# knagrecha/saturn

Hardware: NVIDIA H100
Metric: candidate schedules/sec (higher is better)
Workload: dtype f32

## Files before the change

### saturn_b200/csrc/sb_common.cuh

```cuda
#pragma once
#include <cuda_runtime.h>
#include <stdint.h>

#include "../../include/saturn_b200.h"

#if defined(__CUDA_ARCH__) && (__CUDA_ARCH__ != 900)
#error "saturn_b200 kernels target sm_90a (H100) only"
#endif

namespace sb {

constexpr int kSlots = SB_NSLOT;
constexpr int kWarp = 32;
constexpr int kMaxNodes = SB_MAX_NODES;
constexpr float kSentinel = 1.0e6f;

__device__ __forceinline__ float inf_f() { return __int_as_float(0x7f800000); }

__device__ __forceinline__ uint32_t smem_u32(const void* p) {
  return static_cast<uint32_t>(__cvta_generic_to_shared(p));
}
__device__ __forceinline__ uint32_t cluster_ctarank() {
  uint32_t r;
  asm volatile("mov.u32 %0, %%cluster_ctarank;" : "=r"(r));
  return r;
}
__device__ __forceinline__ void cluster_sync_all() {
  asm volatile("barrier.cluster.arrive.release.aligned;" ::: "memory");
  asm volatile("barrier.cluster.wait.acquire.aligned;" ::: "memory");
}
__device__ __forceinline__ uint32_t cluster_map_shared(uint32_t addr, uint32_t rank) {
  uint32_t r;
  asm volatile("mapa.shared::cluster.u32 %0, %1, %2;" : "=r"(r) : "r"(addr), "r"(rank));
  return r;
}

__device__ __forceinline__ void mbar_init(uint64_t* bar, uint32_t count) {
  asm volatile("mbarrier.init.shared::cta.b64 [%0], %1;" ::"r"(smem_u32(bar)), "r"(count) : "memory");
}
__device__ __forceinline__ void mbar_fence_init() {
  asm volatile("fence.mbarrier_init.release.cluster;" ::: "memory");
}
__device__ __forceinline__ void fence_proxy_async() {
  asm volatile("fence.proxy.async.shared::cta;" ::: "memory");
}
__device__ __forceinline__ void mbar_arrive_expect_tx(uint64_t* bar, uint32_t bytes) {
  asm volatile("mbarrier.arrive.expect_tx.shared::cta.b64 _, [%0], %1;" ::"r"(smem_u32(bar)), "r"(bytes)
               : "memory");
}
__device__ __forceinline__ bool mbar_try_wait(uint64_t* bar, uint32_t parity) {
  uint32_t ok;
  asm volatile(
      "{\n\t.reg .pred p;\n\t"
      "mbarrier.try_wait.parity.shared::cta.b64 p, [%1], %2;\n\t"
      "selp.u32 %0, 1, 0, p;\n\t}"
      : "=r"(ok)
      : "r"(smem_u32(bar)), "r"(parity)
      : "memory");
  return ok != 0;
}
__device__ __forceinline__ void mbar_wait(uint64_t* bar, uint32_t parity) {
  uint32_t spins = 0;
  while (!mbar_try_wait(bar, parity)) {
    if (++spins > (1u << 26)) __trap();
  }
}
__device__ __forceinline__ void tma_bulk_g2s(void* dst_smem, const void* src_gmem, uint32_t bytes,
                                             uint64_t* bar) {
  asm volatile(
      "cp.async.bulk.shared::cluster.global.mbarrier::complete_tx::bytes [%0], [%1], %2, [%3];" ::"r"(
          smem_u32(dst_smem)),
      "l"(src_gmem), "r"(bytes), "r"(smem_u32(bar))
      : "memory");
}

__device__ __forceinline__ void pmov_fma(float& dst, float src, int bit, int one) {
  int d = __float_as_int(dst);
  asm("{\n\t.reg .pred p;\n\tsetp.ne.s32 p, %2, 0;\n\t@p mad.lo.s32 %0, %1, %3, 0;\n\t}"
      : "+r"(d)
      : "r"(__float_as_int(src)), "r"(bit), "r"(one));
  dst = __int_as_float(d);
}
__device__ __forceinline__ void pinf_fma(float& dst, int bit) {
  asm("{\n\t.reg .pred p;\n\tsetp.ne.s32 p, %1, 0;\n\t@p add.f32 %0, %0, 0f7F800000;\n\t}" : "+f"(dst) : "r"(bit));
}
__device__ __forceinline__ float psel(float a, float b, int bit) {
  float r;
  asm("{\n\t.reg .pred p;\n\tsetp.ne.s32 p, %3, 0;\n\tselp.f32 %0, %1, %2, p;\n\t}" : "=f"(r) : "f"(a), "f"(b), "r"(bit));
  return r;
}

__device__ __forceinline__ float fmax3(float a, float b, float c) { return fmaxf(fmaxf(a, b), c); }

template <bool kIntegerStarts, bool kTrackMk = kIntegerStarts>
__device__ __forceinline__ void ls_step(float (&f)[8], float& mk, float& pend, float rt, int km1, int one, int ph) {
  const float INF = inf_f();
  const int b2 = km1 & 4, b1 = km1 & 2, b0 = km1 & 1;
  float x0 = psel(f[4], f[0], b2), x1 = psel(f[5], f[1], b2), x2 = psel(f[6], f[2], b2), x3 = psel(f[7], f[3], b2);
  const float m2 = psel(INF, -0.0f, b2);
  float x4 = f[4] + m2, x5 = f[5] + m2, x6 = f[6] + m2, x7 = f[7] + m2;
  pmov_fma(x0, x2, b1, one); pmov_fma(x1, x3, b1, one); pmov_fma(x2, x4, b1, one); pmov_fma(x3, x5, b1, one);
  pmov_fma(x4, x6, b1, one); pmov_fma(x5, x7, b1, one); pinf_fma(x6, b1); pinf_fma(x7, b1);
  pmov_fma(x0, x1, b0, one); pmov_fma(x1, x2, b0, one); pmov_fma(x2, x3, b0, one); pmov_fma(x3, x4, b0, one);
  pmov_fma(x4, x5, b0, one); pmov_fma(x5, x6, b0, one); pmov_fma(x6, x7, b0, one); pinf_fma(x7, b0);
  const float s = x0;
  float v;
  if (kIntegerStarts) {
    v = s + ceilf(rt);
  } else {
    v = s + rt;
  }
  if (kTrackMk) {
    const float e = kIntegerStarts ? s + rt : v;
    if (ph < 0) mk = fmaxf(mk, e);
    else if (ph == 0) pend = e;
    else mk = fmax3(mk, pend, e);
  }
  f[0] = fmaxf(f[0], fminf(v, x1));
  f[1] = fmaxf(f[1], fminf(v, x2));
  f[2] = fmaxf(f[2], fminf(v, x3));
  f[3] = fmaxf(f[3], fminf(v, x4));
  f[4] = fmaxf(f[4], fminf(v, x5));
  f[5] = fmaxf(f[5], fminf(v, x6));
  f[6] = fmaxf(f[6], fminf(v, x7));
  f[7] = fmaxf(f[7], v);
}

__device__ __forceinline__ unsigned long long pack_key(float mk, uint32_t id) {
  return (static_cast<unsigned long long>(__float_as_uint(mk)) << 32) | id;
}

__device__ __host__ __forceinline__ uint64_t mix64(uint64_t z) {
  z += 0x9e3779b97f4a7c15ull;
  z = (z ^ (z >> 30)) * 0xbf58476d1ce4e5b9ull;
  z = (z ^ (z >> 27)) * 0x94d049bb133111ebull;
  return z ^ (z >> 31);
}
__device__ __host__ __forceinline__ uint64_t rng_u64(uint64_t seed, uint64_t stream, uint64_t ctr) {
  return mix64(mix64(seed ^ (stream * 0xd1342543de82ef95ull)) + ctr * 0x2545f4914f6cdd1dull);
}

}
```

### saturn_b200/csrc/sb_eval.cu

```cuda
#include "sb_lane.cuh"

namespace sb {

struct TileArgs {
  const float* tab;
  int J, SG;
  const uint8_t* opt;
  const uint8_t* prio;
  long long B;
  long long stride_o, stride_p;
  int row_o, row_p;
  int copy_o, copy_p;
  int use_bulk;
  int nodes;
  float* out;
  unsigned long long* best_key;
  uint32_t id_base;
  long long ntiles;
  int one;
  SearchFuse sf;
  XchgPost xp;
};

template <int PB, bool INT, bool STREAM, bool MULTI, bool SEARCH = false, bool TABG = false, int ADDR = 0>
__global__ void __launch_bounds__(STREAM ? 512 : 384, 1) k_eval_tiles(const TileArgs a) {
  static_assert(!(SEARCH && (STREAM || TABG)), "the fused search round runs on shared-memory tiles only");
  static_assert(ADDR == 0 || (!TABG && !MULTI && !SEARCH), "ADDR = 1 needs the table and the opt rows in shared memory");
  extern __shared__ __align__(128) uint8_t smem[];
  const int nw = blockDim.x >> 5;
  const int warp = threadIdx.x >> 5, lane = threadIdx.x & 31;
  const uint32_t tab_bytes = TABG ? 0u : static_cast<uint32_t>(a.J) * a.SG * 4u;
  float* tab_s = reinterpret_cast<float*>(smem);
  uint64_t* bars = reinterpret_cast<uint64_t*>(smem + ((tab_bytes + 15u) & ~15u));
  uint8_t* tiles = reinterpret_cast<uint8_t*>(bars) + (((1 + nw) * 8 + 15) & ~15);
  const uint32_t node_bytes = MULTI ? static_cast<uint32_t>(a.nodes) * 1024u : 0u;
  const uint32_t tile_bytes = 32u * (a.row_o + (STREAM ? 0 : a.row_p)) + node_bytes;
  uint8_t* wbase = tiles + static_cast<size_t>(warp) * tile_bytes;
  float4* node_s = reinterpret_cast<float4*>(wbase);
  uint8_t* tile_o = wbase + node_bytes;
  uint8_t* tile_p = tile_o + 32u * a.row_o;
  uint64_t* bar_tab = bars;
  uint64_t* bar_w = bars + 1 + warp;

  if (threadIdx.x == 0) {
    mbar_init(bar_tab, 1);
    for (int w = 0; w < nw; ++w) mbar_init(bars + 1 + w, 1);
    mbar_fence_init();
  }
  __syncthreads();
  if constexpr (!TABG) {
    if (threadIdx.x == 0) {
      mbar_arrive_expect_tx(bar_tab, tab_bytes);
      const uint8_t* src = reinterpret_cast<const uint8_t*>(a.tab);
      for (uint32_t off = 0; off < tab_bytes; off += 32768u) {
        uint32_t n = min(32768u, tab_bytes - off);
        tma_bulk_g2s(smem + off, src + off, n, bar_tab);
      }
    }
  }

  LaneState<INT, MULTI, ADDR> st;
  if (TABG) st.tab = a.tab;
  else st.tab = tab_s;
  st.SG = a.SG;
  st.one = a.one;
  st.orow = tile_o + lane * a.row_o;
  st.ns = node_s + lane;
  st.orow_s = smem_u32(tile_o + lane * a.row_o);
  st.tab_s = smem_u32(tab_s);
  st.four = static_cast<uint32_t>(a.one) * 4u;

  bool fold_pending = a.xp.counter != nullptr && a.xp.fold_prev && a.xp.seq > 1 && blockIdx.x == 0 && warp == 0;
  unsigned long long pf_seen = 0ull, pf_key = ~0ull;
  auto look_issue = [&]() {
    if (lane < a.xp.x.world) {
      const unsigned long long* slot = a.xp.x.peer[lane] + ((a.xp.seq - 1) & 1ull) * 2;
      asm volatile("ld.acquire.sys.global.u64 %0, [%1];" : "=l"(pf_seen) : "l"(slot + 1) : "memory");
      asm volatile("ld.relaxed.sys.global.u64 %0, [%1];" : "=l"(pf_key) : "l"(slot) : "memory");
    }
  };
  auto fold_keys = [&](unsigned long long k) {
#pragma unroll
    for (int d = 16; d > 0; d >>= 1) {
      const unsigned long long o = __shfl_xor_sync(0xffffffffu, k, d);
      k = o < k ? o : k;
    }
    if (lane == 0) atomicMin(a.best_key, k);
    fold_pending = false;
  };
  auto look_consume = [&]() {
    const unsigned long long want = a.xp.seq - 1;
    const bool ok = lane >= a.xp.x.world || pf_seen >= want;
    if (__all_sync(0xffffffffu, ok)) fold_keys(lane < a.xp.x.world ? pf_key : ~0ull);
  };
  auto try_fold = [&](bool block) {
    const unsigned long long want = a.xp.seq - 1;
    unsigned long long k = ~0ull;
    bool ok = true;
    if (lane < a.xp.x.world) {
      const unsigned long long* slot = a.xp.x.peer[lane] + (want & 1ull) * 2;
      unsigned long long seen;
      unsigned spins = 0;
      for (;;) {
        asm volatile("ld.acquire.sys.global.u64 %0, [%1];" : "=l"(seen) : "l"(slot + 1) : "memory");
        if (seen >= want || !block || ++spins >= (1u << 22)) break;
        __nanosleep(64);
      }
      ok = seen >= want;
      if (ok) asm volatile("ld.relaxed.sys.global.u64 %0, [%1];" : "=l"(k) : "l"(slot) : "memory");
    }
    ok = __all_sync(0xffffffffu, ok);
    if (!ok) {
      if (block && lane == 0) *a.xp.error = 1;
      return;
    }
    fold_keys(k);
  };
  if (fold_pending) look_issue();

  uint32_t phase = 0;
  bool tab_ready = TABG;
  for (long long tile = static_cast<long long>(blockIdx.x) * nw + warp; tile < a.ntiles;
       tile += static_cast<long long>(gridDim.x) * nw) {
    const long long b0 = tile * 32;
    if (!SEARCH && fold_pending) {
      look_consume();
      if (fold_pending) look_issue();
    }
    const long long cand = (SEARCH && a.sf.deal) ? lane * a.ntiles + tile : b0 + lane;
    const bool active = cand < a.B;
    const int nb = SEARCH ? __popc(__ballot_sync(0xffffffffu, active)) : static_cast<int>(min(32ll, a.B - b0));
    const uint8_t* pg = a.prio + cand * a.stride_p;
    __syncwarp();
    PrioChunk q;
    if (a.use_bulk) {
      fence_proxy_async();
      if (lane == 0)
        mbar_arrive_expect_tx(bar_w, static_cast<uint32_t>(nb) * (a.copy_o + (STREAM ? 0 : a.copy_p)));
      __syncwarp();
      if (active) {
        tma_bulk_g2s(tile_o + lane * a.row_o, a.opt + cand * a.stride_o, a.copy_o, bar_w);
        if (!STREAM) tma_bulk_g2s(tile_p + lane * a.row_p, pg, a.copy_p, bar_w);
      }
      if (STREAM && active) q = ld_prio32<true>(pg);
      mbar_wait(bar_w, phase);
      phase ^= 1;
    } else {
      for (int r = 0; r < nb; ++r) {
        const uint8_t* so = a.opt + (b0 + r) * a.stride_o;
        const uint8_t* sp = a.prio + (b0 + r) * a.stride_p;
        for (int x = lane; x < a.J; x += 32) tile_o[r * a.row_o + x] = so[x];
        for (int x = lane; x < a.J * PB; x += 32) tile_p[r * a.row_p + x] = sp[x];
      }
      __syncwarp();
    }
    if (!tab_ready) {
      mbar_wait(bar_tab, 0);
      tab_ready = true;
    }
    auto evaluate = [&](const uint8_t* prio_row_s) -> float {
      st.reset(a.nodes);
      const int J = a.J;
      if (STREAM) {
        constexpr int STEPS = 32 / PB;
        const int nch = (J + STEPS - 1) / STEPS;
        for (int c = 0; c < nch; ++c) {
          PrioChunk nxt = q;
          if (c + 1 < nch) nxt = ld_prio32<true>(pg + (c + 1) * 32);
          if ((c + 1) * STEPS <= J) {
#pragma unroll
            for (int t = 0; t < STEPS; ++t) st.step(prio_at<PB>(q.w, t), t & 1);
          } else {
            const int rem = J - c * STEPS;
#pragma unroll
            for (int t = 0; t < STEPS; ++t)
              if (t < rem) st.step(prio_at<PB>(q.w, t), t & 1);
          }
          q = nxt;
        }
      } else {
        const uint4* prow = reinterpret_cast<const uint4*>(prio_row_s);
        constexpr int STEPS = 16 / PB;
        const int nch = (J + STEPS - 1) / STEPS;
        for (int c = 0; c < nch; ++c) {
          const uint4 p = prow[c];
          const uint32_t w[4] = {p.x, p.y, p.z, p.w};
          if ((c + 1) * STEPS <= J) {
#pragma unroll
            for (int t = 0; t < STEPS; ++t) st.step(prio_at<PB>(w, t), t & 1);
          } else {
            const int rem = J - c * STEPS;
#pragma unroll
            for (int t = 0; t < STEPS; ++t)
              if (t < rem) st.step(prio_at<PB>(w, t), t & 1);
          }
        }
      }
      return st.result();
    };
    [[maybe_unused]] auto eval_from = [&](const uint8_t* prio_row_s, int w0, uint32_t par, bool save,
                                          float* snap_t) -> float {
      const int J = a.J;
      constexpr int STEPS = 16 / PB;
      constexpr int CPW = kSnapPos / STEPS;
      const int nch = (J + STEPS - 1) / STEPS;
      if (w0 == 0) {
        st.reset(a.nodes);
      } else {
        const float* sp = snap_t + (((w0 - 1) * 2 + ((par >> (w0 - 1)) & 1u)) * 9) * 32 + lane;
#pragma unroll
        for (int i = 0; i < 8; ++i) st.f[i] = __ldcg(sp + i * 32);
        st.mk = __ldcg(sp + 8 * 32);
        st.pend = 0.f;
      }
      const uint4* prow = reinterpret_cast<const uint4*>(prio_row_s);
#pragma unroll 1
      for (int c = w0 * CPW; c < nch; ++c) {
        if (save && c > w0 * CPW && (c % CPW) == 0) {
          const int b = c / CPW - 1;
          float* sp = snap_t + ((b * 2 + (((par >> b) & 1u) ^ 1u)) * 9) * 32 + lane;
#pragma unroll
          for (int i = 0; i < 8; ++i) __stcg(sp + i * 32, st.f[i]);
          __stcg(sp + 8 * 32, fmaxf(st.mk, st.pend));
        }
        const uint4 p = prow[c];
        const uint32_t wd[4] = {p.x, p.y, p.z, p.w};
        if ((c + 1) * STEPS <= J) {
#pragma unroll
          for (int t = 0; t < STEPS; ++t) st.step(prio_at<PB>(wd, t), t & 1);
        } else {
          const int rem = J - c * STEPS;
#pragma unroll 1
          for (int t = 0; t < rem; ++t) st.step(PB == 1 ? prio_row_s[c * STEPS + t] : reinterpret_cast<const uint16_t*>(prio_row_s)[c * STEPS + t], -1);
        }
      }
      return st.result();
    };
    if (!SEARCH) {
      float mk = 0.f;
      if (active) {
        mk = evaluate(tile_p + lane * a.row_p);
        a.out[b0 + lane] = mk;
      }
      if (a.best_key != nullptr) fold_best(a.best_key, active, mk, a.id_base + static_cast<uint32_t>(b0 + lane), lane);
    } else {
      const long long c = cand;
      const int rl = active ? lane : 0;
      uint8_t* orow_s = tile_o + rl * a.row_o;
      uint8_t* prow_s = tile_p + rl * a.row_p;
      st.orow = orow_s;
      const uint64_t gid = a.sf.chain_base + static_cast<uint64_t>(c);
      float cm = active ? a.sf.cur_mk[c] : 0.f;
      bool moving = active;
      const bool inc = !MULTI && a.sf.snap != nullptr;
      const bool win = !MULTI && a.sf.win != 0;
      const int nwin = (a.J + kSnapPos - 1) / kSnapPos;
      float* snap_t = inc ? a.sf.snap + static_cast<size_t>(tile) * (static_cast<size_t>(nwin - 1) * 2 * 9 * 32) : nullptr;
      uint32_t par = 0;
      const uint32_t inc_bits = launch_incumbent_bits(a.sf);
#pragma unroll 1
      for (int r = inc ? -1 : 0; r < a.sf.nrounds; ++r) {
        const int round = a.sf.round + r;
        const bool fill = r < 0;
        if (!fill && a.sf.resample_every > 0 && round > 1 && (round - 1) % a.sf.resample_every == 0) {
          const uint64_t rr = rng_u64(a.sf.seed ^ 0x7e57a11ull, gid, static_cast<uint64_t>(round));
          const int rival = static_cast<int>(rr >> 59);
          const float rcm = __shfl_sync(0xffffffffu, cm, rival);
          const bool ractive = (__ballot_sync(0xffffffffu, active) >> rival) & 1u;
          const bool take = moving && ractive && rcm < cm;
          const uint4* so = reinterpret_cast<const uint4*>(tile_o + rival * a.row_o);
          const uint4* sp = reinterpret_cast<const uint4*>(tile_p + rival * a.row_p);
          uint4* go = reinterpret_cast<uint4*>(a.sf.cur_o + c * a.stride_o);
          uint4* gp = reinterpret_cast<uint4*>(a.sf.cur_p + c * a.stride_p);
          for (int i = 0; i * 16 < a.copy_o; ++i) {
            const uint4 v = so[i];
            __syncwarp();
            if (take) { reinterpret_cast<uint4*>(orow_s)[i] = v; go[i] = v; }
            __syncwarp();
          }
          for (int i = 0; i * 16 < a.copy_p; ++i) {
            const uint4 v = sp[i];
            __syncwarp();
            if (take) { reinterpret_cast<uint4*>(prow_s)[i] = v; gp[i] = v; }
            __syncwarp();
          }
          if (inc) {
            const uint32_t rpar = __shfl_sync(0xffffffffu, par, rival);
            constexpr int kBatch = 7;
            for (int b0s = 0; b0s < nwin - 1; b0s += kBatch) {
              float v[kBatch][9];
#pragma unroll
              for (int bb = 0; bb < kBatch; ++bb) {
                const int b = b0s + bb;
                if (take && b < nwin - 1) {
                  const float* src = snap_t + ((b * 2 + ((rpar >> b) & 1u)) * 9) * 32 + rival;
#pragma unroll
                  for (int i = 0; i < 9; ++i) v[bb][i] = __ldcg(src + i * 32);
                }
              }
              __syncwarp();
#pragma unroll
              for (int bb = 0; bb < kBatch; ++bb) {
                const int b = b0s + bb;
                if (take && b < nwin - 1) {
                  float* dst = snap_t + ((b * 2 + ((par >> b) & 1u)) * 9) * 32 + lane;
#pragma unroll
                  for (int i = 0; i < 9; ++i) __stcg(dst + i * 32, v[bb][i]);
                }
              }
              __syncwarp();
            }
          }
          if (take) {
            cm = rcm;
            a.sf.cur_mk[c] = rcm;
          }
        }
        int w0 = 0;
        if (win && !fill) {
          const uint64_t wr = rng_u64(a.sf.seed ^ 0x31d0ull, a.sf.chain_base + static_cast<uint64_t>(a.sf.deal ? tile : b0),
                                      static_cast<uint64_t>(round));
          w0 = draw_window(wr, nwin, a.sf.win_bias);
        }
        Move mv;
        mv.kind = 0; mv.a = mv.b = mv.va = mv.vb = 0;
        if (moving && !fill) {
          if (win) {
            const int p0 = w0 * kSnapPos;
            mv = apply_move_win<PB>(a.sf, round, a.J, gid, orow_s, prow_s, p0, min(kSnapPos, a.J - p0));
          } else {
            mv = apply_move<PB>(a.sf, round, a.J, gid, orow_s, prow_s);
          }
        }
        __syncwarp();
        float mk = 0.f;
        const int trips = (inc && !fill && a.sf.verify_bad != nullptr) ? 2 : 1;
#pragma unroll 1
        for (int trip = 0; trip < trips; ++trip) {
          const float got = eval_from(prow_s, (inc && trip == 0) ? w0 : 0, fill ? ~0u : par, inc && trip == 0, snap_t);
          if (trip == 0) mk = got;
          else if (active && __float_as_uint(got) != __float_as_uint(mk)) atomicAdd(a.sf.verify_bad, 1ull);
        }
        if (fill) continue;
        if (moving) {
          bool acc = mk <= cm;
          const float temp = a.sf.temperature[r];
          if (!acc && temp > 0.f && isfinite(mk)) {
            const uint64_t rr = rng_u64(a.sf.seed, gid, 4ull * round + 3);
            const float u = (static_cast<uint32_t>(rr >> 40) + 0.5f) * (1.0f / 16777216.0f);
            acc = u < __expf(-(mk - cm) / temp);
          }
          if (acc) {
            if (mv.kind != 0) {
              write_back<PB>(mv, orow_s, prow_s, a.sf.cur_o + c * a.stride_o, a.sf.cur_p + c * a.stride_p);
              a.sf.cur_mk[c] = mk;
              cm = mk;
              if (inc) par ^= (w0 + 1 < nwin) ? (~0u << w0) : 0u;
            }
          } else {
            undo_move<PB>(mv, orow_s, prow_s);
            mk = cm;
          }
        }
        if (a.best_key != nullptr) fold_best(a.best_key, active, mk, a.id_base + static_cast<uint32_t>(c), lane);
        if (active && __float_as_uint(mk) < inc_bits) moving = false;
      }
      st.orow = tile_o + lane * a.row_o;
    }
  }
  if (!tab_ready && threadIdx.x == 0) mbar_wait(bar_tab, 0);
  if (!SEARCH && fold_pending) try_fold(true);
  if (SEARCH) {
    if (a.sf.keep.counter != nullptr) keep_best_tail(a.sf);
    return;
  }
  if (a.xp.counter != nullptr) {
    __syncthreads();
    if (threadIdx.x == 0) {
      __threadfence();
      const unsigned done = atomicAdd(a.xp.counter, 1u);
      if (done == gridDim.x - 1) {
        *a.xp.counter = 0;
        __threadfence();
        const unsigned long long k = *reinterpret_cast<volatile unsigned long long*>(a.best_key);
        unsigned long long* slot = a.xp.x.local + (a.xp.seq & 1ull) * 2;
        asm volatile("st.relaxed.sys.global.u64 [%0], %1;" ::"l"(slot), "l"(k) : "memory");
        asm volatile("st.release.sys.global.u64 [%0], %1;" ::"l"(slot + 1), "l"(a.xp.seq) : "memory");
      }
    }
  }
}

struct GenericArgs {
  const float* tab;
  int J, SG;
  const uint8_t* opt;
  const uint8_t* prio;
  long long B;
  long long stride_o, stride_p;
  float* out;
  unsigned long long* best_key;
  uint32_t id_base;
  int tab_in_smem;
  int nodes;
  int one;
};

template <int PB, bool INT, bool MULTI>
__global__ void __launch_bounds__(128) k_eval_generic(const GenericArgs a) {
  extern __shared__ __align__(128) uint8_t smem[];
  const float* tab = a.tab;
  const uint32_t node_bytes = MULTI ? static_cast<uint32_t>(a.nodes) * 1024u : 0u;
  float4* node_s = reinterpret_cast<float4*>(smem) + (threadIdx.x >> 5) * (node_bytes / 16);
  if (a.tab_in_smem) {
    float* tab_s = reinterpret_cast<float*>(smem + (blockDim.x >> 5) * node_bytes);
    const int n = a.J * a.SG;
    for (int i = threadIdx.x; i < n; i += blockDim.x) tab_s[i] = a.tab[i];
    __syncthreads();
    tab = tab_s;
  }
  const int lane = threadIdx.x & 31;
  LaneState<INT, MULTI> st;
  st.tab = tab;
  st.SG = a.SG;
  st.one = a.one;
  st.ns = node_s + lane;
  const long long nthreads = static_cast<long long>(gridDim.x) * blockDim.x;
  const long long Bpad = (a.B + 31) & ~31ll;
  for (long long b = static_cast<long long>(blockIdx.x) * blockDim.x + threadIdx.x; b < Bpad; b += nthreads) {
    const bool active = b < a.B;
    float mk = 0.f;
    if (active) {
      st.orow = a.opt + b * a.stride_o;
      const uint8_t* prow = a.prio + b * a.stride_p;
      st.reset(a.nodes);
      constexpr int BATCH = 16;
      int i = 0;
      for (; i + BATCH <= a.J; i += BATCH) {
        int js[BATCH], os[BATCH];
        float rts[BATCH];
#pragma unroll
        for (int t = 0; t < BATCH; ++t) js[t] = PB == 1 ? prow[i + t] : reinterpret_cast<const uint16_t*>(prow)[i + t];
#pragma unroll
        for (int t = 0; t < BATCH; ++t) os[t] = st.lookup_opt(js[t]);
#pragma unroll
        for (int t = 0; t < BATCH; ++t) rts[t] = st.lookup_rt(js[t], os[t]);
#pragma unroll
        for (int t = 0; t < BATCH; ++t) st.step_resolved(os[t], rts[t], t & 1);
      }
      for (; i < a.J; ++i) st.step(PB == 1 ? prow[i] : reinterpret_cast<const uint16_t*>(prow)[i]);
      mk = st.result();
      a.out[b] = mk;
    }
    if (a.best_key != nullptr) fold_best(a.best_key, active, mk, a.id_base + static_cast<uint32_t>(b), lane);
  }
}

struct FullArgs {
  const float* tab;
  int J, SG;
  const uint8_t* opt;
  const uint8_t* prio;
  long long B;
  long long stride_o, stride_p;
  int nodes;
  float* out;
  float* start;
  uint32_t* slotmask;
};

template <int PB, bool INT>
__global__ void __launch_bounds__(128) k_eval_full(const FullArgs a) {
  const long long nthreads = static_cast<long long>(gridDim.x) * blockDim.x;
  const bool multi = a.nodes > 1;
  for (long long b = static_cast<long long>(blockIdx.x) * blockDim.x + threadIdx.x; b < a.B; b += nthreads) {
    const uint8_t* orow = a.opt + b * a.stride_o;
    const uint8_t* prow = a.prio + b * a.stride_p;
    float ready[kMaxNodes * kSlots];
    for (int g = 0; g < a.nodes * kSlots; ++g) ready[g] = 0.f;
    float mk = 0.f;
    for (int i = 0; i < a.J; ++i) {
      const int j = PB == 1 ? prow[i] : reinterpret_cast<const uint16_t*>(prow)[i];
      const int o = orow[j];
      const int k = (o & 7) + 1;
      const int node = multi ? (o >> 3) : 0;
      const float rt = __ldg(a.tab + static_cast<size_t>(j) * a.SG + (multi ? (o & 7) : o));
      float* rd = ready + node * kSlots;
      uint32_t taken = 0;
      float s = 0.f;
      for (int q = 0; q < k; ++q) {
        int best = -1;
        float bv = 0.f;
        for (int g = 0; g < kSlots; ++g) {
          const bool free_slot = ((taken >> g) & 1u) == 0u;
          if (free_slot && (best < 0 || rd[g] < bv)) {
            best = g;
            bv = rd[g];
          }
        }
        taken |= 1u << best;
        s = bv;
      }
      const float hold = (INT && isfinite(rt)) ? ceilf(rt) : rt;
      const float nxt = s + hold;
      for (int g = 0; g < kSlots; ++g)
        if ((taken >> g) & 1u) rd[g] = nxt;
      mk = fmaxf(mk, s + rt);
      if (a.start) a.start[b * a.J + j] = s;
      if (a.slotmask) a.slotmask[b * a.J + j] = (static_cast<uint32_t>(node) << 16) | taken;
    }
    if (a.out) a.out[b] = mk;
  }
}

__global__ void k_validate(const float* tab, int J, int SG, int nodes, const uint8_t* opt, const uint8_t* prio, int pb,
                           long long B, long long stride_o, long long stride_p, unsigned long long* bad, int by_pos) {
  const int lane = threadIdx.x & 31;
  const long long warp = (static_cast<long long>(blockIdx.x) * blockDim.x + threadIdx.x) >> 5;
  const long long nwarps = (static_cast<long long>(gridDim.x) * blockDim.x) >> 5;
  extern __shared__ uint32_t seen_all[];
  const int words = (J + 31) / 32;
  uint32_t* seen = seen_all + (threadIdx.x >> 5) * words;
  for (long long b = warp; b < B; b += nwarps) {
    for (int w = lane; w < words; w += 32) seen[w] = 0;
    __syncwarp();
    bool ok = true;
    const uint8_t* orow = opt + b * stride_o;
    const uint8_t* prow = prio + b * stride_p;
    for (int i = lane; i < J; i += 32) {
      const int j = pb == 1 ? prow[i] : reinterpret_cast<const uint16_t*>(prow)[i];
      if (j >= J) {
        ok = false;
      } else {
        const uint32_t old = atomicOr(&seen[j >> 5], 1u << (j & 31));
        if (old & (1u << (j & 31))) ok = false;
      }
      int o = orow[i];
      if (nodes > 1) {
        if ((o >> 3) >= nodes) ok = false;
        o &= 7;
      }
      const int job = by_pos ? (j < J ? j : 0) : i;
      if (o >= SG || !isfinite(tab[static_cast<size_t>(job) * SG + o])) ok = false;
    }
    ok = __all_sync(0xffffffffu, ok);
    if (!ok && lane == 0) atomicAdd(bad, 1ull);
    __syncwarp();
  }
}

static int round_row(int bytes) {
  int r16 = (bytes + 15) / 16;
  if ((r16 & 1) == 0) r16 += 1;
  return r16 * 16;
}

int plan_tiles(const Device& dev, int J, int SG, int pb, bool stream, int nodes, TilePlan* tp, bool tab_global) {
  tp->row_o = round_row(J);
  tp->row_p = round_row(J * pb);
  tp->copy_o = (J + 15) & ~15;
  tp->copy_p = (J * pb + 15) & ~15;
  const size_t tab_bytes = tab_global ? 0 : ((static_cast<size_t>(J) * SG * 4 + 15) & ~size_t(15));
  const size_t per_warp = 32u * static_cast<size_t>(tp->row_o + (stream ? 0 : tp->row_p)) +
                          (nodes > 1 ? static_cast<size_t>(nodes) * 1024u : 0u);
  int nw = stream ? 16 : 12;
  while (nw > 0 && tab_bytes + 16 * ((1 + nw + 1) / 2) + nw * per_warp > dev.smem_optin) --nw;
  tp->warps = nw;
  tp->smem = tab_bytes + (((1 + nw) * 8 + 15) & ~15) + nw * per_warp;
  return nw;
}

template <int PB, bool INT, bool STREAM, bool MULTI, bool TABG = false, int ADDR = 0>
static cudaError_t launch_tiles(const Device& dev, const TileArgs& a, const TilePlan& tp, cudaStream_t st) {
  auto kern = k_eval_tiles<PB, INT, STREAM, MULTI, false, TABG, ADDR>;
  cudaError_t e = cudaFuncSetAttribute(kern, cudaFuncAttributeMaxDynamicSharedMemorySize, static_cast<int>(tp.smem));
  if (e != cudaSuccess) return e;
  long long ctas = (a.ntiles + tp.warps - 1) / tp.warps;
  int grid = static_cast<int>(ctas < dev.sm_count ? ctas : dev.sm_count);
  kern<<<grid, tp.warps * 32, tp.smem, st>>>(a);
  return cudaGetLastError();
}

template <int PB, bool INT>
static cudaError_t dispatch_tiles(const Device& dev, const TileArgs& a, const TilePlan& tp, bool stream, bool multi,
                                  cudaStream_t st) {
  if (stream) {
    return multi ? launch_tiles<PB, INT, true, true>(dev, a, tp, st) : launch_tiles<PB, INT, true, false>(dev, a, tp, st);
  }
  return multi ? launch_tiles<PB, INT, false, true>(dev, a, tp, st) : launch_tiles<PB, INT, false, false>(dev, a, tp, st);
}

template <int PB, bool INT, bool MULTI>
static cudaError_t launch_generic(const Device& dev, const GenericArgs& a0, cudaStream_t st) {
  GenericArgs a = a0;
  auto kern = k_eval_generic<PB, INT, MULTI>;
  const size_t tab_bytes = static_cast<size_t>(a.J) * a.SG * 4;
  size_t smem = MULTI ? static_cast<size_t>(4) * a.nodes * 1024u : 0u;
  a.tab_in_smem = 0;
  if (tab_bytes <= dev.smem_optin / 2) {
    a.tab_in_smem = 1;
    smem += tab_bytes;
  }
  if (smem > 0) {
    cudaError_t e = cudaFuncSetAttribute(kern, cudaFuncAttributeMaxDynamicSharedMemorySize, static_cast<int>(smem));
    if (e != cudaSuccess) return e;
  }
  long long blocks = (a.B + 127) / 128;
  long long cap = static_cast<long long>(dev.sm_count) * 8;
  int grid = static_cast<int>(blocks < cap ? blocks : cap);
  if (grid < 1) grid = 1;
  kern<<<grid, 128, smem, st>>>(a);
  return cudaGetLastError();
}

cudaError_t eval_launch(const Device& dev, const EvalCall& c, cudaStream_t st, int* path_used) {
  if (c.B <= 0) return cudaSuccess;
  const int pb = c.J <= 256 ? 1 : 2;
  const bool ints = (c.flags & SB_FLAG_INTEGER_STARTS) != 0;
  const bool multi = c.nodes > 1;
  const bool bulk_ok = (c.stride_o % 16 == 0) && (c.stride_p % 16 == 0) &&
                       (reinterpret_cast<uintptr_t>(c.opt) % 16 == 0) && (reinterpret_cast<uintptr_t>(c.prio) % 16 == 0);
  const bool stream_ok = bulk_ok && (c.stride_p % 32 == 0) && (reinterpret_cast<uintptr_t>(c.prio) % 32 == 0) &&
                         !(c.flags & 0x40000000u);
  TilePlan tp;
  int nw = 0;
  bool stream = false, tabg = false;
  if (!c.force_generic) {
    if (stream_ok) {
      nw = plan_tiles(dev, c.J, c.SG, pb, true, c.nodes, &tp);
      stream = nw >= 2 && c.stride_o >= tp.copy_o && c.stride_p >= ((c.J * pb + 31) & ~31);
      if (!stream && !multi) {
        nw = plan_tiles(dev, c.J, c.SG, pb, true, c.nodes, &tp, true);
        stream = tabg = nw >= 2 && c.stride_o >= tp.copy_o && c.stride_p >= ((c.J * pb + 31) & ~31);
      }
    }
    if (!stream) nw = plan_tiles(dev, c.J, c.SG, pb, false, c.nodes, &tp);
  }
  if (nw >= 2) {
    TileArgs a;
    a.tab = c.tab; a.J = c.J; a.SG = c.SG; a.opt = c.opt; a.prio = c.prio; a.B = c.B;
    a.stride_o = c.stride_o; a.stride_p = c.stride_p;
    a.row_o = tp.row_o; a.row_p = tp.row_p; a.copy_o = tp.copy_o; a.copy_p = tp.copy_p;
    a.use_bulk = stream || (bulk_ok && (c.stride_o >= tp.copy_o) && (c.stride_p >= tp.copy_p));
    a.nodes = c.nodes;
    a.out = c.out; a.best_key = c.best_key; a.id_base = c.id_base;
    a.ntiles = (c.B + 31) / 32;
    a.one = 1;
    a.xp = c.xp;
    if (path_used) *path_used = tabg ? 4 : (stream ? 3 : (a.use_bulk ? 2 : 1));
    if (tabg) {
      if (pb == 1) return ints ? launch_tiles<1, true, true, false, true>(dev, a, tp, st) : launch_tiles<1, false, true, false, true>(dev, a, tp, st);
      return ints ? launch_tiles<2, true, true, false, true>(dev, a, tp, st) : launch_tiles<2, false, true, false, true>(dev, a, tp, st);
    }
    if (pb == 1 && stream && !multi && !(c.flags & 0x02000000u))
      return ints ? launch_tiles<1, true, true, false, false, 1>(dev, a, tp, st) : launch_tiles<1, false, true, false, false, 1>(dev, a, tp, st);
    if (pb == 1) return ints ? dispatch_tiles<1, true>(dev, a, tp, stream, multi, st) : dispatch_tiles<1, false>(dev, a, tp, stream, multi, st);
    return ints ? dispatch_tiles<2, true>(dev, a, tp, stream, multi, st) : dispatch_tiles<2, false>(dev, a, tp, stream, multi, st);
  }
  GenericArgs g;
  g.tab = c.tab; g.J = c.J; g.SG = c.SG; g.opt = c.opt; g.prio = c.prio; g.B = c.B;
  g.stride_o = c.stride_o; g.stride_p = c.stride_p; g.out = c.out; g.best_key = c.best_key;
  g.id_base = c.id_base; g.tab_in_smem = 0; g.nodes = c.nodes; g.one = 1;
  if (path_used) *path_used = 0;
  if (multi) {
    if (pb == 1) return ints ? launch_generic<1, true, true>(dev, g, st) : launch_generic<1, false, true>(dev, g, st);
    return ints ? launch_generic<2, true, true>(dev, g, st) : launch_generic<2, false, true>(dev, g, st);
  }
  if (pb == 1) return ints ? launch_generic<1, true, false>(dev, g, st) : launch_generic<1, false, false>(dev, g, st);
  return ints ? launch_generic<2, true, false>(dev, g, st) : launch_generic<2, false, false>(dev, g, st);
}

template <int PB, bool INT>
static cudaError_t dispatch_search(const Device& dev, const TileArgs& a, const TilePlan& tp, bool multi,
                                   cudaStream_t st) {
  auto launch = [&](auto kern) {
    cudaError_t e = cudaFuncSetAttribute(kern, cudaFuncAttributeMaxDynamicSharedMemorySize, static_cast<int>(tp.smem));
    if (e != cudaSuccess) return e;
    long long ctas = (a.ntiles + tp.warps - 1) / tp.warps;
    int grid = static_cast<int>(ctas < dev.sm_count ? ctas : dev.sm_count);
    kern<<<grid, tp.warps * 32, tp.smem, st>>>(a);
    return cudaGetLastError();
  };
  if (multi) return launch(k_eval_tiles<PB, INT, false, true, true>);
  return launch(k_eval_tiles<PB, INT, false, false, true>);
}

int search_round_mode(const Device& dev, int J, int SG, int nodes) {
  const int pb = J <= 256 ? 1 : 2;
  TilePlan tp;
  return plan_tiles(dev, J, SG, pb, false, nodes, &tp) >= 8 ? 2 : 0;
}

cudaError_t search_round_launch(const Device& dev, const EvalCall& c, const SearchFuse& sf, cudaStream_t st) {
  if (c.B <= 0) return cudaSuccess;
  const int pb = c.J <= 256 ? 1 : 2;
  const bool ints = (c.flags & SB_FLAG_INTEGER_STARTS) != 0;
  const bool bulk_ok = (c.stride_o % 16 == 0) && (c.stride_p % 16 == 0) &&
                       (reinterpret_cast<uintptr_t>(c.opt) % 16 == 0) && (reinterpret_cast<uintptr_t>(c.prio) % 16 == 0);
  TilePlan tp;
  if (search_round_mode(dev, c.J, c.SG, c.nodes) == 0 || !bulk_ok) return cudaErrorNotSupported;
  plan_tiles(dev, c.J, c.SG, pb, false, c.nodes, &tp);
  if (c.stride_o < tp.copy_o || c.stride_p < tp.copy_p) return cudaErrorNotSupported;
  TileArgs a;
  a.tab = c.tab; a.J = c.J; a.SG = c.SG; a.opt = c.opt; a.prio = c.prio; a.B = c.B;
  a.stride_o = c.stride_o; a.stride_p = c.stride_p;
  a.row_o = tp.row_o; a.row_p = tp.row_p; a.copy_o = tp.copy_o; a.copy_p = tp.copy_p;
  a.use_bulk = 1;
  a.nodes = c.nodes;
  a.out = nullptr; a.best_key = c.best_key; a.id_base = c.id_base;
  a.ntiles = (c.B + 31) / 32;
  a.one = 1;
  a.sf = sf;
  if (pb == 1)
    return ints ? dispatch_search<1, true>(dev, a, tp, c.nodes > 1, st)
                : dispatch_search<1, false>(dev, a, tp, c.nodes > 1, st);
  return ints ? dispatch_search<2, true>(dev, a, tp, c.nodes > 1, st)
              : dispatch_search<2, false>(dev, a, tp, c.nodes > 1, st);
}

cudaError_t eval_full_launch(const Device& dev, const EvalCall& c, float* start, uint32_t* slotmask, cudaStream_t st) {
  if (c.B <= 0) return cudaSuccess;
  const int pb = c.J <= 256 ? 1 : 2;
  const bool ints = (c.flags & SB_FLAG_INTEGER_STARTS) != 0;
  FullArgs a;
  a.tab = c.tab; a.J = c.J; a.SG = c.SG; a.opt = c.opt; a.prio = c.prio; a.B = c.B;
  a.stride_o = c.stride_o; a.stride_p = c.stride_p; a.nodes = c.nodes < 1 ? 1 : c.nodes;
  a.out = c.out; a.start = start; a.slotmask = slotmask;
  long long blocks = (c.B + 127) / 128;
  long long cap = static_cast<long long>(dev.sm_count) * 16;
  int grid = static_cast<int>(blocks < cap ? blocks : cap);
  if (pb == 1) {
    if (ints) k_eval_full<1, true><<<grid, 128, 0, st>>>(a);
    else k_eval_full<1, false><<<grid, 128, 0, st>>>(a);
  } else {
    if (ints) k_eval_full<2, true><<<grid, 128, 0, st>>>(a);
    else k_eval_full<2, false><<<grid, 128, 0, st>>>(a);
  }
  return cudaGetLastError();
}

cudaError_t validate_launch(const Device& dev, const EvalCall& c, unsigned long long* bad, cudaStream_t st, bool by_pos) {
  if (c.B <= 0) return cudaSuccess;
  const int pb = c.J <= 256 ? 1 : 2;
  const int words = (c.J + 31) / 32;
  const int threads = 128;
  size_t smem = static_cast<size_t>(threads / 32) * words * 4;
  long long blocks = (c.B + 3) / 4;
  long long cap = static_cast<long long>(dev.sm_count) * 8;
  int grid = static_cast<int>(blocks < cap ? blocks : cap);
  k_validate<<<grid, threads, smem, st>>>(c.tab, c.J, c.SG, c.nodes, c.opt, c.prio, pb, c.B, c.stride_o, c.stride_p, bad,
                                          by_pos ? 1 : 0);
  return cudaGetLastError();
}

}
```

### saturn_b200/csrc/sb_lane.cuh

```cuda
#pragma once
#include "sb_internal.h"

namespace sb {

struct PrioChunk {
  uint32_t w[8];
};
template <bool kReadOnly>
__device__ __forceinline__ PrioChunk ld_prio32(const uint8_t* p) {
  PrioChunk c;
  if (kReadOnly) {
    asm volatile("ld.global.nc.L1::no_allocate.v4.u32 {%0,%1,%2,%3}, [%8];\n\t"
                 "ld.global.nc.L1::no_allocate.v4.u32 {%4,%5,%6,%7}, [%8+16];"
                 : "=r"(c.w[0]), "=r"(c.w[1]), "=r"(c.w[2]), "=r"(c.w[3]), "=r"(c.w[4]), "=r"(c.w[5]), "=r"(c.w[6]),
                   "=r"(c.w[7])
                 : "l"(p));
  } else {
    asm volatile("ld.global.L1::no_allocate.v4.u32 {%0,%1,%2,%3}, [%8];\n\t"
                 "ld.global.L1::no_allocate.v4.u32 {%4,%5,%6,%7}, [%8+16];"
                 : "=r"(c.w[0]), "=r"(c.w[1]), "=r"(c.w[2]), "=r"(c.w[3]), "=r"(c.w[4]), "=r"(c.w[5]), "=r"(c.w[6]),
                   "=r"(c.w[7])
                 : "l"(p)
                 : "memory");
  }
  return c;
}

template <bool INT, bool MULTI, int ADDR = 0>
struct LaneState {
  float f[8];
  float mk;
  float pend;
  const uint8_t* orow;
  const float* tab;
  int SG;
  int one;
  uint32_t orow_s, tab_s, four;
  float4* ns;
  int cur;

  __device__ __forceinline__ void reset(int nodes) {
#pragma unroll
    for (int i = 0; i < 8; ++i) f[i] = 0.f;
    mk = 0.f;
    pend = 0.f;
    cur = 0;
    if (MULTI) {
      const float4 z = make_float4(0.f, 0.f, 0.f, 0.f);
      for (int n = 0; n < 2 * nodes; ++n) ns[n * 32] = z;
    }
  }
  __device__ __forceinline__ void switch_node(int n) {
    if (n != cur) {
      float4* old = ns + (2 * cur) * 32;
      old[0] = make_float4(f[0], f[1], f[2], f[3]);
      old[32] = make_float4(f[4], f[5], f[6], f[7]);
      const float4* slot = ns + (2 * n) * 32;
      const float4 lo = slot[0], hi = slot[32];
      f[0] = lo.x; f[1] = lo.y; f[2] = lo.z; f[3] = lo.w;
      f[4] = hi.x; f[5] = hi.y; f[6] = hi.z; f[7] = hi.w;
      cur = n;
    }
  }
  __device__ __forceinline__ int lookup_opt(int j) const { return orow[j]; }
  __device__ __forceinline__ float lookup_rt(int j, int o) const {
    return MULTI ? tab[j * 8 + (o & 7)] : tab[j * SG + o];
  }
  __device__ __forceinline__ void step_resolved(int o, float rt, int ph = -1) {
    if (!MULTI) {
      ls_step<INT>(f, mk, pend, rt, o & 7, one, ph);
    } else {
      switch_node(o >> 3);
      ls_step<INT, true>(f, mk, pend, rt, o & 7, one, ph);
    }
  }
  __device__ __forceinline__ void step(int j, int ph = -1) {
    if (!MULTI && ADDR == 1) {
      uint32_t oa, o, idx, ta;
      float rt;
      asm("mad.lo.u32 %0, %1, %2, %3;" : "=r"(oa) : "r"(j), "r"(one), "r"(orow_s));
      asm("ld.shared.u8 %0, [%1];" : "=r"(o) : "r"(oa));
      asm("mad.lo.u32 %0, %1, %2, %3;" : "=r"(idx) : "r"(j), "r"(SG), "r"(o));
      asm("mad.lo.u32 %0, %1, %2, %3;" : "=r"(ta) : "r"(idx), "r"(four), "r"(tab_s));
      asm("ld.shared.f32 %0, [%1];" : "=f"(rt) : "r"(ta));
      ls_step<INT>(f, mk, pend, rt, static_cast<int>(o & 7u), one, ph);
      return;
    }
    const int o = orow[j];
    if (!MULTI) {
      const float rt = tab[j * SG + o];
      ls_step<INT>(f, mk, pend, rt, o & 7, one, ph);
    } else {
      const int col = o & 7;
      const float rt = tab[j * 8 + col];
      switch_node(o >> 3);
      ls_step<INT, true>(f, mk, pend, rt, col, one, ph);
    }
  }
  __device__ __forceinline__ float result() const { return (INT || MULTI) ? fmaxf(mk, pend) : f[7]; }
};

template <int PB>
__device__ __forceinline__ int prio_at(const uint32_t* w, int t) {
  if (PB == 1) return static_cast<int>(__byte_perm(w[t >> 2], 0u, 0x4440u + (t & 3)));
  return static_cast<int>(__byte_perm(w[t >> 1], 0u, (t & 1) ? 0x4432u : 0x4410u));
}

__device__ __forceinline__ bool fold_best(unsigned long long* best_key, bool active, float mk, uint32_t id, int lane) {
  const uint32_t bits = active ? __float_as_uint(mk) : 0xffffffffu;
  const uint32_t mn = __reduce_min_sync(0xffffffffu, bits);
  const uint32_t who = __ballot_sync(0xffffffffu, bits == mn);
  bool lowered = false;
  if (lane == __ffs(who) - 1 && active) {
    const unsigned long long key = pack_key(mk, id);
    if (key < *reinterpret_cast<volatile unsigned long long*>(best_key)) lowered = key < atomicMin(best_key, key);
  }
  return lowered;
}

__device__ __forceinline__ uint32_t launch_incumbent_bits(const SearchFuse& sf) {
  return sf.keep.keys != nullptr
             ? static_cast<uint32_t>(*reinterpret_cast<volatile unsigned long long*>(sf.keep.keys + 1) >> 32)
             : 0u;
}

__device__ __forceinline__ void keep_best_tail(const SearchFuse& sf) {
  __threadfence();
  __syncthreads();
  int mine = 0;
  if (threadIdx.x == 0) {
    const unsigned done = atomicAdd(sf.keep.counter, 1u);
    mine = done == gridDim.x - 1;
    if (mine) *sf.keep.counter = 0;
  }
  if (!__syncthreads_or(mine) || threadIdx.x >= 32) return;
  __threadfence();
  const int lane = threadIdx.x;
  const unsigned long long key = *reinterpret_cast<volatile unsigned long long*>(sf.keep.keys);
  if ((key >> 32) >= (*reinterpret_cast<volatile unsigned long long*>(sf.keep.keys + 1) >> 32)) return;
  const long long c = static_cast<long long>(((key & 0xffffffffull) - (sf.chain_base & 0xffffffffull)) & 0xffffffffull);
  if (c >= sf.keep.chains) return;
  const uint4* so = reinterpret_cast<const uint4*>(sf.cur_o + c * sf.keep.stride_o);
  const uint4* sp = reinterpret_cast<const uint4*>(sf.cur_p + c * sf.keep.stride_p);
  for (int i = lane; i * 16 < sf.keep.stride_o; i += 32) reinterpret_cast<uint4*>(sf.keep.best_o)[i] = __ldcg(so + i);
  for (int i = lane; i * 16 < sf.keep.stride_p; i += 32) reinterpret_cast<uint4*>(sf.keep.best_p)[i] = __ldcg(sp + i);
  __syncwarp();
  if (lane == 0) sf.keep.keys[1] = key;
}

struct Move {
  int kind;
  int a, b;
  int va, vb;
};

__device__ __forceinline__ uint32_t bounded32(uint64_t r, uint32_t n) {
  return static_cast<uint32_t>((static_cast<uint64_t>(static_cast<uint32_t>(r >> 32)) * n) >> 32);
}

template <int PB>
__device__ __forceinline__ int smem_prio_ld(const uint8_t* row, int i) {
  return PB == 1 ? row[i] : reinterpret_cast<const uint16_t*>(row)[i];
}
template <int PB>
__device__ __forceinline__ void smem_prio_st(uint8_t* row, int i, int v) {
  if (PB == 1) row[i] = static_cast<uint8_t>(v);
  else reinterpret_cast<uint16_t*>(row)[i] = static_cast<uint16_t>(v);
}

template <int PB>
__device__ __forceinline__ Move apply_move(const SearchFuse& sf, int round, int J, uint64_t gid, uint8_t* orow,
                                           uint8_t* prow) {
  Move m;
  m.kind = 0; m.a = 0; m.b = 0; m.va = 0; m.vb = 0;
  const uint64_t r0 = rng_u64(sf.seed, gid, 4ull * round + 0);
  const uint64_t r1 = rng_u64(sf.seed, gid, 4ull * round + 1);
  const uint64_t r2 = rng_u64(sf.seed, gid, 4ull * round + 2);
  const uint32_t kind = bounded32(r0, 100);
  if (sf.nodes > 1 && kind >= 85) {
    const int j = bounded32(r1, J);
    const uint8_t curv = orow[j];
    int nn = bounded32(r2, sf.nodes - 1);
    if (nn >= (curv >> 3)) ++nn;
    orow[j] = static_cast<uint8_t>((curv & 7) | (nn << 3));
    m.kind = 1; m.a = j; m.va = curv;
    return m;
  }
  if (kind < 30) {
    const int j = bounded32(r1, J);
    const int n = sf.nvalid[j];
    if (n > 1) {
      const int pick = bounded32(r2, n - 1);
      const uint8_t curv = orow[j];
      const uint8_t node_bits = sf.nodes > 1 ? (curv & 0xf8) : 0;
      const uint8_t cur_opt = sf.nodes > 1 ? (curv & 7) : curv;
      uint8_t nv = sf.vopt[j * kSlots + pick];
      if (nv == cur_opt) nv = sf.vopt[j * kSlots + n - 1];
      orow[j] = nv | node_bits;
      m.kind = 1; m.a = j; m.va = curv;
      return m;
    }
  }
  if (J < 2) return m;
  const int a = bounded32(r1, J);
  if (kind < 70) {
    int b = bounded32(r2, J - 1);
    if (b >= a) ++b;
    const int va = smem_prio_ld<PB>(prow, a), vb = smem_prio_ld<PB>(prow, b);
    smem_prio_st<PB>(prow, a, vb);
    smem_prio_st<PB>(prow, b, va);
    m.kind = 2; m.a = a; m.b = b; m.va = va; m.vb = vb;
    return m;
  }
  const int span = J - 1 < 48 ? J - 1 : 48;
  int d = 1 + static_cast<int>(bounded32(r2, 2 * span));
  int b = d <= span ? a + d : a - (d - span);
  if (b < 0) b = 0;
  if (b > J - 1) b = J - 1;
  if (b == a) return m;
  const int va = smem_prio_ld<PB>(prow, a);
  if (a < b) {
    for (int i = a; i < b; ++i) smem_prio_st<PB>(prow, i, smem_prio_ld<PB>(prow, i + 1));
  } else {
    for (int i = a; i > b; --i) smem_prio_st<PB>(prow, i, smem_prio_ld<PB>(prow, i - 1));
  }
  smem_prio_st<PB>(prow, b, va);
  m.kind = 3; m.a = a < b ? a : b; m.b = a < b ? b : a; m.va = a; m.vb = b;
  return m;
}

__device__ __forceinline__ int draw_window(uint64_t r, int nwin, int bias) {
  if (bias == 0) return static_cast<int>(bounded32(r, nwin));
  const uint32_t tot = static_cast<uint32_t>(nwin) * (nwin + 1) / 2;
  const uint32_t t = bounded32(r, tot);
  int w = static_cast<int>((sqrtf(8.f * static_cast<float>(t) + 1.f) - 1.f) * 0.5f);
  while (static_cast<uint32_t>(w + 1) * (w + 2) / 2 <= t) ++w;
  while (static_cast<uint32_t>(w) * (w + 1) / 2 > t) --w;
  return w;
}

template <int PB>
__device__ __forceinline__ Move apply_move_win(const SearchFuse& sf, int round, int J, uint64_t gid, uint8_t* orow,
                                               uint8_t* prow, int w0, int wlen) {
  Move m;
  m.kind = 0; m.a = 0; m.b = 0; m.va = 0; m.vb = 0;
  const uint64_t r0 = rng_u64(sf.seed, gid, 4ull * round + 0);
  const uint64_t r1 = rng_u64(sf.seed, gid, 4ull * round + 1);
  const uint64_t r2 = rng_u64(sf.seed, gid, 4ull * round + 2);
  const uint32_t kind = bounded32(r0, 100);
  const int a = w0 + static_cast<int>(bounded32(r1, wlen));
  if (kind < 30) {
    const int j = smem_prio_ld<PB>(prow, a);
    const int n = sf.nvalid[j];
    if (n > 1) {
      const int pick = bounded32(r2, n - 1);
      const uint8_t curv = orow[j];
      uint8_t nv = sf.vopt[j * kSlots + pick];
      if (nv == curv) nv = sf.vopt[j * kSlots + n - 1];
      orow[j] = nv;
      m.kind = 1; m.a = j; m.va = curv;
      return m;
    }
  }
  const int tail = J - w0;
  if (tail < 2) return m;
  if (kind < 70) {
    int b = w0 + static_cast<int>(bounded32(r2, tail - 1));
    if (b >= a) ++b;
    const int va = smem_prio_ld<PB>(prow, a), vb = smem_prio_ld<PB>(prow, b);
    smem_prio_st<PB>(prow, a, vb);
    smem_prio_st<PB>(prow, b, va);
    m.kind = 2; m.a = a; m.b = b; m.va = va; m.vb = vb;
    return m;
  }
  const int span = J - 1 < 48 ? J - 1 : 48;
  const uint32_t dd = bounded32(r2, 2 * span);
  int b = a + 1 + static_cast<int>(dd >> 1);
  if (b > J - 1) b = J - 1;
  if (b == a) return m;
  if (dd & 1) {
    const int va = smem_prio_ld<PB>(prow, a);
    for (int i = a; i < b; ++i) smem_prio_st<PB>(prow, i, smem_prio_ld<PB>(prow, i + 1));
    smem_prio_st<PB>(prow, b, va);
    m.va = a; m.vb = b;
  } else {
    const int vb = smem_prio_ld<PB>(prow, b);
    for (int i = b; i > a; --i) smem_prio_st<PB>(prow, i, smem_prio_ld<PB>(prow, i - 1));
    smem_prio_st<PB>(prow, a, vb);
    m.va = b; m.vb = a;
  }
  m.kind = 3; m.a = a; m.b = b;
  return m;
}

template <int PB>
__device__ __forceinline__ void undo_move(const Move& m, uint8_t* orow, uint8_t* prow) {
  if (m.kind == 1) {
    orow[m.a] = static_cast<uint8_t>(m.va);
  } else if (m.kind == 2) {
    smem_prio_st<PB>(prow, m.a, m.va);
    smem_prio_st<PB>(prow, m.b, m.vb);
  } else if (m.kind == 3) {
    const int from = m.vb, to = m.va;
    const int job = smem_prio_ld<PB>(prow, from);
    if (from < to) {
      for (int i = from; i < to; ++i) smem_prio_st<PB>(prow, i, smem_prio_ld<PB>(prow, i + 1));
    } else {
      for (int i = from; i > to; --i) smem_prio_st<PB>(prow, i, smem_prio_ld<PB>(prow, i - 1));
    }
    smem_prio_st<PB>(prow, to, job);
  }
}

template <int PB>
__device__ __forceinline__ void write_back(const Move& m, const uint8_t* orow, const uint8_t* prow, uint8_t* go,
                                           uint8_t* gp) {
  if (m.kind == 1) {
    go[m.a] = orow[m.a];
  } else if (m.kind == 2) {
    if (PB == 1) { gp[m.a] = static_cast<uint8_t>(m.vb); gp[m.b] = static_cast<uint8_t>(m.va); }
    else {
      reinterpret_cast<uint16_t*>(gp)[m.a] = static_cast<uint16_t>(m.vb);
      reinterpret_cast<uint16_t*>(gp)[m.b] = static_cast<uint16_t>(m.va);
    }
  } else if (m.kind == 3) {
    for (int i = m.a; i <= m.b; ++i) {
      if (PB == 1) gp[i] = prow[i];
      else reinterpret_cast<uint16_t*>(gp)[i] = reinterpret_cast<const uint16_t*>(prow)[i];
    }
  }
}

template <int PB>
__device__ __forceinline__ void patch_chunk(PrioChunk& q, int c, int pos, int val) {
  constexpr int STEPS = 32 / PB;
  if (pos / STEPS != c) return;
  const int t = pos % STEPS;
  const int widx = PB == 1 ? (t >> 2) : (t >> 1);
  const int sh = PB == 1 ? (t & 3) * 8 : (t & 1) * 16;
  const uint32_t mask = (PB == 1 ? 0xffu : 0xffffu) << sh;
  const uint32_t ins = static_cast<uint32_t>(val) << sh;
#pragma unroll
  for (int i = 0; i < 8; ++i)
    if (i == widx) q.w[i] = (q.w[i] & ~mask) | ins;
}

}
```

Baseline: 1.718 billion.

## Software-pipeline shared-memory opt/runtime gathers ahead of scheduling steps in stream path

For the streaming ADDR=1 path, the per-step dependent shared-memory loads (opt byte, then runtime table entry) are resolved in batches of eight one batch ahead of the list-scheduling steps that consume them, so load latency overlaps with the ls_step arithmetic. It also replaces the float fmax3 on the makespan with an integer three-way max (__vimax3_s32), which is valid for non-negative floats. The batching raises register pressure and adds a separate tail loop for partial chunks. The integer max would give wrong results if negative values ever appeared.

```diff
diff --git a/saturn_b200/csrc/sb_common.cuh b/saturn_b200/csrc/sb_common.cuh
--- a/saturn_b200/csrc/sb_common.cuh
+++ b/saturn_b200/csrc/sb_common.cuh
@@ -90,7 +90,9 @@
   return r;
 }
 
-__device__ __forceinline__ float fmax3(float a, float b, float c) { return fmaxf(fmaxf(a, b), c); }
+__device__ __forceinline__ float fmax3_mk(float mk, float b, float c) {
+  return __int_as_float(__vimax3_s32(__float_as_int(mk), __float_as_int(b), __float_as_int(c)));
+}
 
 template <bool kIntegerStarts, bool kTrackMk = kIntegerStarts>
 __device__ __forceinline__ void ls_step(float (&f)[8], float& mk, float& pend, float rt, int km1, int one, int ph) {
@@ -114,7 +116,7 @@
     const float e = kIntegerStarts ? s + rt : v;
     if (ph < 0) mk = fmaxf(mk, e);
     else if (ph == 0) pend = e;
-    else mk = fmax3(mk, pend, e);
+    else mk = fmax3_mk(mk, pend, e);
   }
   f[0] = fmaxf(f[0], fminf(v, x1));
   f[1] = fmaxf(f[1], fminf(v, x2));
diff --git a/saturn_b200/csrc/sb_eval.cu b/saturn_b200/csrc/sb_eval.cu
--- a/saturn_b200/csrc/sb_eval.cu
+++ b/saturn_b200/csrc/sb_eval.cu
@@ -161,7 +161,48 @@
     auto evaluate = [&](const uint8_t* prio_row_s) -> float {
       st.reset(a.nodes);
       const int J = a.J;
-      if (STREAM) {
+      if constexpr (STREAM && ADDR == 1) {
+        constexpr int STEPS = 32;
+        constexpr int kBatch = 8;
+        const int nch = (J + STEPS - 1) / STEPS, nfull = J / STEPS;
+        uint32_t ob[kBatch];
+        float rb[kBatch];
+        auto resolve = [&](const uint32_t* w) {
+          int js[kBatch];
+#pragma unroll
+          for (int i = 0; i < kBatch; ++i) js[i] = prio_at<1>(w, i);
+#pragma unroll
+          for (int i = 0; i < kBatch; ++i) ob[i] = st.gather_opt(js[i]);
+#pragma unroll
+          for (int i = 0; i < kBatch; ++i) rb[i] = st.gather_rt(js[i], ob[i]);
+        };
+        if (nfull > 0) resolve(q.w);
+        for (int c = 0; c < nfull; ++c) {
+          PrioChunk nxt = q;
+          if (c + 1 < nch) nxt = ld_prio32<true>(pg + (c + 1) * 32);
+          const bool ahead = c + 1 < nfull;
+          uint32_t head[kBatch / 4];
+#pragma unroll
+          for (int i = 0; i < kBatch / 4; ++i) head[i] = ahead ? nxt.w[i] : q.w[i];
+#pragma unroll
+          for (int b = 0; b < STEPS / kBatch; ++b) {
+            uint32_t oc[kBatch];
+            float rc[kBatch];
+#pragma unroll
+            for (int i = 0; i < kBatch; ++i) { oc[i] = ob[i]; rc[i] = rb[i]; }
+            resolve(b + 1 < STEPS / kBatch ? q.w + (b + 1) * (kBatch / 4) : head);
+#pragma unroll
+            for (int i = 0; i < kBatch; ++i) st.step_resolved(static_cast<int>(oc[i]), rc[i], i & 1);
+          }
+          q = nxt;
+        }
+        if (nfull < nch) {
+          const int rem = J - nfull * STEPS;
+#pragma unroll
+          for (int t = 0; t < STEPS; ++t)
+            if (t < rem) st.step(prio_at<1>(q.w, t), t & 1);
+        }
+      } else if (STREAM) {
         constexpr int STEPS = 32 / PB;
         const int nch = (J + STEPS - 1) / STEPS;
         for (int c = 0; c < nch; ++c) {
diff --git a/saturn_b200/csrc/sb_lane.cuh b/saturn_b200/csrc/sb_lane.cuh
--- a/saturn_b200/csrc/sb_lane.cuh
+++ b/saturn_b200/csrc/sb_lane.cuh
@@ -74,16 +74,24 @@
       ls_step<INT, true>(f, mk, pend, rt, o & 7, one, ph);
     }
   }
+  __device__ __forceinline__ uint32_t gather_opt(int j) const {
+    uint32_t oa, o;
+    asm("mad.lo.u32 %0, %1, %2, %3;" : "=r"(oa) : "r"(j), "r"(one), "r"(orow_s));
+    asm("ld.shared.u8 %0, [%1];" : "=r"(o) : "r"(oa));
+    return o;
+  }
+  __device__ __forceinline__ float gather_rt(int j, uint32_t o) const {
+    uint32_t idx, ta;
+    float rt;
+    asm("mad.lo.u32 %0, %1, %2, %3;" : "=r"(idx) : "r"(j), "r"(SG), "r"(o));
+    asm("mad.lo.u32 %0, %1, %2, %3;" : "=r"(ta) : "r"(idx), "r"(four), "r"(tab_s));
+    asm("ld.shared.f32 %0, [%1];" : "=f"(rt) : "r"(ta));
+    return rt;
+  }
   __device__ __forceinline__ void step(int j, int ph = -1) {
     if (!MULTI && ADDR == 1) {
-      uint32_t oa, o, idx, ta;
-      float rt;
-      asm("mad.lo.u32 %0, %1, %2, %3;" : "=r"(oa) : "r"(j), "r"(one), "r"(orow_s));
-      asm("ld.shared.u8 %0, [%1];" : "=r"(o) : "r"(oa));
-      asm("mad.lo.u32 %0, %1, %2, %3;" : "=r"(idx) : "r"(j), "r"(SG), "r"(o));
-      asm("mad.lo.u32 %0, %1, %2, %3;" : "=r"(ta) : "r"(idx), "r"(four), "r"(tab_s));
-      asm("ld.shared.f32 %0, [%1];" : "=f"(rt) : "r"(ta));
-      ls_step<INT>(f, mk, pend, rt, static_cast<int>(o & 7u), one, ph);
+      const uint32_t o = gather_opt(j);
+      ls_step<INT>(f, mk, pend, gather_rt(j, o), static_cast<int>(o & 7u), one, ph);
       return;
     }
     const int o = orow[j];
```

After: 1.822 billion (median of 6 runs). +6.0%, better.
